# yas-sim/pyopenvino

Hardware: AMD Instinct MI355X
Metric: images/sec googlenet-v1 fp32 @batch256 (higher is better)
Workload: dtype f32

## Files before the change

include/pvhip.h:

```cpp
#ifndef PVHIP_H
#define PVHIP_H

#include <stddef.h>
#include <stdint.h>

#ifdef __cplusplus
extern "C" {
#endif

#define PVHIP_OK            0
#define PVHIP_EHIP         -1
#define PVHIP_EINVAL       -2
#define PVHIP_ENOTINIT     -3
#define PVHIP_ECOMM        -4
#define PVHIP_EUNSUPPORTED -5

#define PVHIP_ABI_VERSION   19

int         pvhip_abi_version(void);
const char* pvhip_last_error(void);
int         pvhip_device_count(int* count);
int         pvhip_init(int device);
int         pvhip_settings_reload(void);
int         pvhip_shutdown(void);
// ... 275 lines not shown
                                       int pad_top, int pad_left, int pad_bottom, int pad_right, int size, float alpha, float beta, float bias,
                                       int k_out, const float* conv_bias, int act);
int    pvhip_conv2d_f16_stem_supported(int c, int h, int w, int k_out, int kh, int kw, int sh, int sw, int pad_top, int pad_left, int oh, int ow);
size_t pvhip_conv2d_f16_stem_pack_elems(int k_out);
int    pvhip_conv2d_f16_stem_pack(const float* w_oihw, float* wf, int k_out);
int    pvhip_conv2d_f16_stem(const float* xp, const float* wf, void* yb, int n, int hp, int wp, int k_out, int oh, int ow,
                             const float* bias, int act);
int    pvhip_conv2d_f16_stem_direct_supported(int c, int h, int w, int k_out, int kh, int kw, int sh, int sw, int pad_top, int pad_left, int oh, int ow);
int    pvhip_conv2d_f16_stem_direct_pack(const float* w_oihw, float* wf, int k_out);
int    pvhip_conv2d_f16_stem_direct(const float* x, const float* wf, void* yb, int n, int h, int w, int k_out, int oh, int ow,
                                    const float* pre_add, const float* bias, int act);
int    pvhip_conv2d_stem_f32_supported(int c, int h, int w, int k_out, int kh, int kw, int sh, int sw, int pad_top, int pad_left, int oh, int ow);
size_t pvhip_conv2d_stem_f32_pack_elems(int k_out);
int    pvhip_conv2d_stem_f32_pack(const float* w_oihw, float* wf, int k_out);
int    pvhip_conv2d_stem_f32(const float* xp, const float* wf, float* y, int n, int hp, int wp, int k_out, int oh, int ow,
                             const float* bias, int act, float act_lo, float act_hi);
int    pvhip_conv2d_stem_direct_supported(int c, int h, int w, int k_out, int kh, int kw, int sh, int sw, int pad_top, int pad_left, int oh, int ow);
int    pvhip_conv2d_stem_direct_f32(const float* x, const float* wf, float* y, int n, int h, int w, int k_out, int oh, int ow,
                                    const float* pre_add, const float* bias, int act, float act_lo, float act_hi);
int    pvhip_conv2d_stem_direct_pool_supported(int n, int c, int h, int w, int k_out, int kh, int kw, int sh, int sw, int pad_top, int pad_left,
                                               int oh, int ow, int poh, int pow);
int    pvhip_conv2d_stem_direct_pool_f32(const float* x, const float* wf, float* y, float* yp, int n, int h, int w, int k_out, int oh, int ow,
                                         int poh, int pow, const float* pre_add, const float* bias, int act, float act_lo, float act_hi);
int    pvhip_conv2d_stem_wino_supported(int c, int h, int w, int k_out, int kh, int kw, int sh, int sw, int pad_top, int pad_left, int oh, int ow);
long   pvhip_conv2d_stem_wino_pack_elems(void);
int    pvhip_conv2d_stem_wino_pack(const float* w_oihw, float* u, int k_out);
int    pvhip_conv2d_stem_wino_f32(const float* x, const float* u, float* y, int n, int h, int w, int k_out, int oh, int ow,
                                  const float* pre_add, const float* bias, int act, float act_lo, float act_hi);
int    pvhip_avgpool_c8(const void* x, float* y, int n, int c, int h, int w, int oh, int ow, int kh, int kw, int sh, int sw);
int    pvhip_lrn_maxpool3x3_c8_supported(int h, int w, int oh, int ow, int sh, int sw, int pad_top, int pad_left, int size);
int    pvhip_lrn_maxpool3x3_c8(const void* x, void* y, int n, int c, int h, int w, int size, float alpha, float beta, float bias,
                               int oh, int ow, int sh, int sw, int pad_top, int pad_left, int pad_bottom, int pad_right);
int    pvhip_conv2d_f16_c8(const void* xb, const float* wf, float* y,
                           int n, int c, int h, int w, int k_out, int kh, int kw,
                           const float* bias, int act,
                           int out_channel_offset, int out_channels_total,
                           float act_lo, float act_hi);

int pvhip_dwconv2d_f32(const float* x, const float* w, float* y, int n, int g, int h, int wdt,
                       int kh, int kw, int oh, int ow, int sh, int sw, int pad_top, int pad_left,
                       const float* bias, int act, float act_lo, float act_hi);

int pvhip_detection_output_f32(const float* loc, const float* conf, const float* priors, float* out, int n,
                               int num_priors, int num_classes, int records_per_image, float confidence_threshold,
                               float nms_threshold, int code_type_center_size, int variance_encoded_in_target,
                               int clip_before_nms, int clip_after_nms);
// ... 144 lines not shown
```

pyopenvino_amd/csrc/pvhip_stem.hip:

```cpp
#include <type_traits>

#include "pvhip_common.h"

using namespace pvhip;

namespace {

typedef float    floatx4 __attribute__((ext_vector_type(4)));
typedef unsigned uintx4 __attribute__((ext_vector_type(4)));
typedef float    floatx2 __attribute__((ext_vector_type(2)));

constexpr int kC = 3, kKH = 7, kKW = 7, kST = 2, kPad = 3;
constexpr int kTR    = 4;
constexpr int kRows  = kST * (kTR - 1) + kKH;
constexpr int kLdsRow = 256;
constexpr int kCopies = kC * kRows;
constexpr int kBufBytes = kCopies * kLdsRow * 4;
constexpr int kTaps  = kC * kKH * kKW;
constexpr int kSteps = (kTaps + 3) / 4;
constexpr int kNG    = 7;
constexpr int kWaves = 2 * kTR;
constexpr int kThreads = kWaves * kWave;
constexpr bool kTransposeStores = true;
constexpr int kTsPitch = 116;
// ... 6 lines not shown
constexpr int kPoolLdsBytes = (kCarryBase + 64 * kHpCols) * 4;

struct StemArgs {
    const float* xp;
    const float* wf;
    float*       y;
    const float* bias;
    const float* pre_add;
    int N, HP, WP, OH, OW, K;
    int tiles_per_image, tiles;
    unsigned x_bytes, y_bytes;
    int act;
    float act_lo, act_hi;
    int tstores;
    float*   yp;
    int      POH, POW;
    unsigned yp_bytes;
};

__device__ __forceinline__ float lds_read_f32(unsigned addr) {
    return *reinterpret_cast<const __attribute__((address_space(3))) float*>(addr);
}

template <int ABL, bool DIRECT, bool POOL = false>
__global__ __launch_bounds__(kThreads, 1) void conv_stem_f32_kernel(StemArgs a) {
    static_assert(!POOL || (DIRECT && ABL == 0 && kTransposeStores), "the pooled output rides on the whole-row stores of the DIRECT form");
    extern __shared__ __attribute__((aligned(1024))) float stem_lds[];
    const int tid  = threadIdx.x;
    const int lane = tid & (kWave - 1);
    const int wid  = __builtin_amdgcn_readfirstlane(tid / kWave);
    const int hf = wid & 1, wr = wid >> 1;
    const int l15 = lane & 15, kq = lane >> 4;

    const int g_ = (int)gridDim.x, b_ = (int)blockIdx.x;
    const int per = a.tiles / g_, extra = a.tiles - per * g_;
    int       tile = b_ * per + min(b_, extra);
    const int tile_end = tile + per + (b_ < extra ? 1 : 0);
    if (tile >= tile_end) return;
    const int  tile_stop = tile_end + ((POOL && tile_end % a.tiles_per_image != 0) ? 1 : 0);
    bool       have_carry = false;

    const __amdgpu_buffer_rsrc_t xr = __builtin_amdgcn_make_buffer_rsrc(const_cast<float*>(a.xp), 0, a.x_bytes, 0x00020000);
    const __amdgpu_buffer_rsrc_t yr = __builtin_amdgcn_make_buffer_rsrc(a.y, 0, a.y_bytes, 0x00020000);

    float w[kSteps][2];
    {
        const float* const wp = a.wf + (size_t)hf * kSteps * 2 * kWave + lane;
#pragma unroll
        for (int m = 0; m < kSteps; ++m) {
// ... 111 lines not shown
        }
        lds_dma_wait_all();
        if (POOL) __syncthreads();
        if (ABL == 1) {
            floatx4 sum = acc[0][0];
#pragma unroll
            for (int g = 0; g < kNG; ++g) sum += acc[g][1] + (g ? acc[g][0] : acc[g][1]);
            if (sum[0] == 12345.678f) __builtin_amdgcn_raw_buffer_store_b128(__builtin_bit_cast(uintx4, sum), yr, (unsigned)(tid * 16), 0, 0);
        } else {
            const int img = tile / a.tiles_per_image;
            const int oy  = (tile - img * a.tiles_per_image) * kTR + wr;
            const unsigned plane = (unsigned)(a.OH * a.OW * 4);
            const unsigned rowb  = (unsigned)(((img * a.K + ch0) * a.OH + oy) * a.OW * 4 + 16 * kq);
            const bool rowok = oy < a.OH && !(POOL && tile >= tile_end);
            if (a.bias != nullptr) {
#pragma unroll
                for (int g = 0; g < kNG; ++g)
#pragma unroll
                    for (int t = 0; t < 2; ++t)
#pragma unroll
                        for (int r = 0; r < 4; ++r) acc[g][t][r] = acc[g][t][r] + bias_l[t];
            }
            auto store_all = [&]() {
                if (kTransposeStores && (POOL || a.tstores != 0)) {
                    float* const tl = stem_lds + kTsBase + wid * kTsWave;
                    const int c2 = lane / 28, q = lane - 28 * c2;
                    float* const hp0 = stem_lds + buf * (kCopies * kLdsRow) + 4 + wid * (16 * kHpCols);
                    int qe = q;
                    if (POOL) asm volatile("" : "+v"(qe));
                    qe = 4 * qe + 4 < a.OW ? 4 * qe + 4 : 4 * qe + 3;
#pragma unroll
                    for (int t = 0; t < 2; ++t) {
#pragma unroll
                        for (int g = 0; g < kNG; ++g) *reinterpret_cast<floatx4*>(tl + l15 * kTsPitch + 16 * g + 4 * kq) = acc[g][t];
                        floatx2 hp[8];
#pragma unroll
                        for (int p = 0; p < 8; ++p) {
                            const int ch = 32 * hf + 16 * t + 2 * p + c2;
                            const floatx4 v = *reinterpret_cast<const floatx4*>(tl + (2 * p + (c2 & 1)) * kTsPitch + 4 * q);
                            if (POOL) {
                                const float e = tl[(2 * p + (c2 & 1)) * kTsPitch + qe];
                                hp[p] = floatx2{max3_nan(v[0], v[1], v[2]), max3_nan(v[2], v[3], e)};
                            }
                            const bool ok = rowok && c2 < 2 && ch < a.K && 4 * q < a.OW;
                            const unsigned vo = ok ? (unsigned)(((img * a.K + ch) * a.OH + oy) * a.OW * 4 + 16 * q) : kOob;
                            __builtin_amdgcn_raw_buffer_store_b128(__builtin_bit_cast(uintx4, v), yr, vo, 0, 0);
// ... 403 lines not shown
                           {0.0f, 0.0f, 0.0f, 1.0f}};
    const int total = 4 * 3 * 36 * kWave;
    for (int e = blockIdx.x * blockDim.x + threadIdx.x; e < total; e += gridDim.x * blockDim.x) {
        const int lane = e & 63, p = (e >> 6) % 36, s = ((e >> 6) / 36) % 3, kg = (e >> 6) / 108;
        const int k = 16 * kg + (lane & 15), gq = lane >> 4, py = gq >> 1, px = gq & 1, pi = p / 6, pj = p - 6 * pi;
        float sum = 0.0f;
        if (k < K) {
            float row[4];
            for (int aa = 0; aa < 4; ++aa) {
                float r = 0.0f;
                for (int bb = 0; bb < 4; ++bb) {
                    const int ky = 2 * aa + py, kx = 2 * bb + px;
                    const float wv = (ky < kKH && kx < kKW) ? w[((size_t)(k * kC + s) * kKH + ky) * kKW + kx] : 0.0f;
                    r = __builtin_fmaf(wv, G[pj][bb], r);
                }
                row[aa] = r;
            }
            for (int aa = 0; aa < 4; ++aa) sum = __builtin_fmaf(G[pi][aa], row[aa], sum);
        }
        u[e] = sum;
    }
}

}

extern "C" {

int pvhip_conv2d_stem_f32_supported(int c, int h, int w, int k_out, int kh, int kw, int sh, int sw, int pad_top, int pad_left, int oh, int ow) {
    if (c != kC || kh != kKH || kw != kKW || sh != kST || sw != kST || pad_top != kPad || pad_left != kPad || k_out <= 0 || k_out > 64) return 0;
    if (h <= 0 || w <= 0 || oh <= 0 || ow <= 0 || ow > 16 * kNG || ow % 4 != 0) return 0;
    const int wp = (kST * (ow - 1) + kKW + 3) / 4 * 4;
    if (wp > kLdsRow || wp < w + kPad) return 0;
    return wp;
}

size_t pvhip_conv2d_stem_f32_pack_elems(int k_out) {
    if (k_out <= 0 || k_out > 64) return 0;
    return (size_t)2 * kSteps * 2 * kWave;
}

int pvhip_conv2d_stem_f32_pack(const float* w_oihw, float* wf, int k_out) {
    PVHIP_REQUIRE_INIT();
    PVHIP_CHECK_ARG(w_oihw != nullptr && wf != nullptr && k_out > 0 && k_out <= 64);
    hipLaunchKernelGGL(conv_stem_f32_pack_kernel, dim3(grid_for((size_t)2 * kSteps * 2 * kWave)), dim3(kBlock), 0, state().stream, w_oihw, wf, k_out);
    PVHIP_LAUNCH_CHECK();
    return PVHIP_OK;
// ... 43 lines not shown
    a.tiles_per_image = (oh + kTR - 1) / kTR;
    const long tiles = (long)n * a.tiles_per_image;
    if (tiles > 0x3fffffffL) return fail(PVHIP_EUNSUPPORTED, "pvhip_conv2d_stem_direct_f32: too many tiles");
    a.tiles = (int)tiles;
    a.x_bytes = (unsigned)in_b; a.y_bytes = (unsigned)out_b;
    a.act = act; a.act_lo = act_lo; a.act_hi = act_hi;
    return stem_launch<true>(a, tiles);
}

int pvhip_conv2d_stem_direct_pool_supported(int n, int c, int h, int w, int k_out, int kh, int kw, int sh, int sw, int pad_top, int pad_left, int oh, int ow,
                                            int poh, int pow) {
    if (!pvhip_conv2d_stem_direct_supported(c, h, w, k_out, kh, kw, sh, sw, pad_top, pad_left, oh, ow)) return 0;
    if (oh < 3 || ow < 4 || poh != (oh - 3 + 1) / 2 + 1 || pow != ow / 2) return 0;
    if (n < 0) return 0;
    if (n > 0) {
        const long tiles = (long)n * ((oh + kTR - 1) / kTR);
        if (tiles < (long)kPoolMinTiles * kNumCU) return 0;
    }
    return 1;
}

int pvhip_conv2d_stem_direct_pool_f32(const float* x, const float* wf, float* y, float* yp, int n, int h, int w, int k_out, int oh, int ow, int poh, int pow,
                                      const float* pre_add, const float* bias, int act, float act_lo, float act_hi) {
    PVHIP_REQUIRE_INIT();
    PVHIP_CHECK_ARG(n >= 0 && k_out > 0 && k_out <= 64 && h > 0 && w > 0 && oh > 0 && ow > 0 && act >= 0 && act <= 2);
    if (!pvhip_conv2d_stem_direct_pool_supported(0, kC, h, w, k_out, kKH, kKW, kST, kST, kPad, kPad, oh, ow, poh, pow))
        return fail(PVHIP_EUNSUPPORTED, "pvhip_conv2d_stem_direct_pool_f32: shape outside the kernel (ask pvhip_conv2d_stem_direct_pool_supported first)");
    const unsigned long long in_b = (unsigned long long)n * kC * h * w * 4ull, out_b = (unsigned long long)n * k_out * oh * ow * 4ull;
    if (in_b >= (1ull << 31) || out_b >= (1ull << 31)) return fail(PVHIP_EUNSUPPORTED, "pvhip_conv2d_stem_direct_pool_f32: tensor too large");
    if (n == 0) return PVHIP_OK;
    PVHIP_CHECK_ARG(x != nullptr && wf != nullptr && y != nullptr && yp != nullptr);
    StemArgs a;
    a.xp = x; a.wf = wf; a.y = y; a.bias = bias; a.pre_add = pre_add;
    a.N = n; a.HP = h; a.WP = w; a.OH = oh; a.OW = ow; a.K = k_out;
    a.tiles_per_image = (oh + kTR - 1) / kTR;
    const long tiles = (long)n * a.tiles_per_image;
    if (tiles > 0x3fffffffL) return fail(PVHIP_EUNSUPPORTED, "pvhip_conv2d_stem_direct_pool_f32: too many tiles");
    a.tiles = (int)tiles;
    a.x_bytes = (unsigned)in_b; a.y_bytes = (unsigned)out_b;
    a.act = act; a.act_lo = act_lo; a.act_hi = act_hi;
    a.tstores = 1;
    a.yp = yp; a.POH = poh; a.POW = pow; a.yp_bytes = (unsigned)((unsigned long long)n * k_out * poh * pow * 4ull);
    const int grid = (int)(tiles < kNumCU ? tiles : kNumCU);
    static bool attr_set = false;
    if (!attr_set) {
        PVHIP_HIP(hipFuncSetAttribute(reinterpret_cast<const void*>(conv_stem_f32_kernel<0, true, true>), hipFuncAttributeMaxDynamicSharedMemorySize, kPoolLdsBytes));
        attr_set = true;
    }
    hipLaunchKernelGGL((conv_stem_f32_kernel<0, true, true>), dim3((unsigned)grid), dim3(kThreads), (size_t)kPoolLdsBytes, state().stream, a);
    PVHIP_LAUNCH_CHECK();
    return PVHIP_OK;
}

int pvhip_conv2d_stem_wino_supported(int c, int h, int w, int k_out, int kh, int kw, int sh, int sw, int pad_top, int pad_left, int oh, int ow) {
    if (c != kC || kh != kKH || kw != kKW || sh != kST || sw != kST || pad_top != kPad || pad_left != kPad || k_out <= 0 || k_out > 64 || k_out % 16 != 0) return 0;
    if (h < 2 || w < 4 || h % 2 != 0 || w % 4 != 0 || w > 224 || oh != h / 2 || ow != w / 2) return 0;
    return 1;
}

long pvhip_conv2d_stem_wino_pack_elems(void) { return 4L * 3 * 36 * kWave; }

int pvhip_conv2d_stem_wino_pack(const float* w_oihw, float* u, int k_out) {
    PVHIP_REQUIRE_INIT();
    PVHIP_CHECK_ARG(w_oihw != nullptr && u != nullptr && k_out > 0 && k_out <= 64);
    hipLaunchKernelGGL(conv_stem_wino_pack_kernel, dim3(grid_for((size_t)4 * 3 * 36 * kWave)), dim3(kBlock), 0, state().stream, w_oihw, u, k_out);
    PVHIP_LAUNCH_CHECK();
    return PVHIP_OK;
}

int pvhip_conv2d_stem_wino_f32(const float* x, const float* u, float* y, int n, int h, int w, int k_out, int oh, int ow, const float* pre_add,
                               const float* bias, int act, float act_lo, float act_hi) {
    PVHIP_REQUIRE_INIT();
    PVHIP_CHECK_ARG(n >= 0 && act >= 0 && act <= 2);
    if (!pvhip_conv2d_stem_wino_supported(kC, h, w, k_out, kKH, kKW, kST, kST, kPad, kPad, oh, ow))
// ... 29 lines not shown
```

pyopenvino_amd/device.py:

```python
import ctypes
import os
import threading
import weakref

import numpy as np

_HERE = os.path.dirname(os.path.abspath(__file__))
LIB_PATH = os.path.join(_HERE, 'libpvhip.so')
DIAG_LIB_PATH = os.path.join(_HERE, 'libpvhip_diag.so')
if os.environ.get('PVHIP_LIBRARY'):
    LIB_PATH = os.path.abspath(os.environ['PVHIP_LIBRARY'])

MAX_RANK = 6
MAX_CONCAT = 16
UNIQUE_ID_BYTES = 128

_c = ctypes
_i64p = _c.POINTER(_c.c_int64)
_fp = _c.c_void_p

SIGNATURES = {
    'pvhip_abi_version': (_c.c_int, []),
    'pvhip_last_error': (_c.c_char_p, []),
    'pvhip_device_count': (_c.c_int, [_c.POINTER(_c.c_int)]),
# ... 90 lines not shown
    'pvhip_conv2d_f16_stem_supported': (_c.c_int, [_c.c_int] * 12),
    'pvhip_conv2d_f16_stem_pack_elems': (_c.c_size_t, [_c.c_int]),
    'pvhip_conv2d_f16_stem_pack': (_c.c_int, [_fp, _fp, _c.c_int]),
    'pvhip_conv2d_f16_stem': (_c.c_int, [_fp, _fp, _c.c_void_p] + [_c.c_int] * 6 + [_fp, _c.c_int]),
    'pvhip_conv2d_f16_stem_direct_supported': (_c.c_int, [_c.c_int] * 12),
    'pvhip_conv2d_f16_stem_direct_pack': (_c.c_int, [_fp, _fp, _c.c_int]),
    'pvhip_conv2d_f16_stem_direct': (_c.c_int, [_fp, _fp, _c.c_void_p] + [_c.c_int] * 6 + [_fp, _fp, _c.c_int]),
    'pvhip_conv2d_f16_dma_c8': (_c.c_int, [_fp, _fp, _c.c_void_p] + [_c.c_int] * 13 + [_fp, _c.c_int]),
    'pvhip_conv2d_f16_c8': (_c.c_int, [_c.c_void_p, _fp, _fp] + [_c.c_int] * 7 + [_fp, _c.c_int, _c.c_int, _c.c_int, _c.c_float, _c.c_float]),
    'pvhip_conv2d_kernel_kind': (_c.c_int, [_c.c_int] * 13),
    'pvhip_conv2d_form': (_c.c_int, [_c.c_int] * 14 + [_c.POINTER(_c.c_int)]),
    'pvhip_conv2d_stem_f32_supported': (_c.c_int, [_c.c_int] * 12),
    'pvhip_conv2d_stem_f32_pack_elems': (_c.c_size_t, [_c.c_int]),
    'pvhip_conv2d_stem_f32_pack': (_c.c_int, [_fp, _fp, _c.c_int]),
    'pvhip_conv2d_stem_f32': (_c.c_int, [_fp, _fp, _fp] + [_c.c_int] * 6 + [_fp, _c.c_int, _c.c_float, _c.c_float]),
    'pvhip_conv2d_stem_direct_supported': (_c.c_int, [_c.c_int] * 12),
    'pvhip_conv2d_stem_wino_supported': (_c.c_int, [_c.c_int] * 12),
    'pvhip_conv2d_stem_wino_pack_elems': (_c.c_long, []),
    'pvhip_conv2d_stem_wino_pack': (_c.c_int, [_fp, _fp, _c.c_int]),
    'pvhip_conv2d_stem_wino_f32': (_c.c_int, [_fp, _fp, _fp] + [_c.c_int] * 6 + [_fp, _fp, _c.c_int, _c.c_float, _c.c_float]),
    'pvhip_conv2d_stem_direct_f32': (_c.c_int, [_fp, _fp, _fp] + [_c.c_int] * 6 + [_fp, _fp, _c.c_int, _c.c_float, _c.c_float]),
    'pvhip_conv2d_stem_direct_pool_supported': (_c.c_int, [_c.c_int] * 15),
    'pvhip_conv2d_stem_direct_pool_f32': (_c.c_int, [_fp, _fp, _fp, _fp] + [_c.c_int] * 8 + [_fp, _fp, _c.c_int, _c.c_float, _c.c_float]),
    'pvhip_lrn_conv1x1_supported': (_c.c_int, [_c.c_int] * 4 + [_c.c_float] * 2 + [_c.c_int]),
    'pvhip_lrn_conv1x1_f32': (_c.c_int, [_fp, _fp, _fp] + [_c.c_int] * 4 + [_c.c_float] * 3 + [_c.c_int, _fp, _c.c_int, _c.c_float, _c.c_float]),
    'pvhip_conv2d_pooled_supported': (_c.c_int, [_c.c_int] * 5),
    'pvhip_conv2d_pooled_f32': (_c.c_int, [_fp, _fp, _fp] + [_c.c_int] * 5 + [_fp, _c.c_int, _c.c_int, _c.c_int, _c.c_float, _c.c_float]),
    'pvhip_conv2d_pooled_f16': (_c.c_int, [_fp, _fp, _fp] + [_c.c_int] * 5 + [_fp, _c.c_int, _c.c_int, _c.c_int, _c.c_float, _c.c_float]),
    'pvhip_conv2d_multi_supported': (_c.c_int, [_c.c_int] * 8),
    'pvhip_conv2d_multi_f32': (_c.c_int, [_fp, _fp] + [_c.c_int] * 12 + [_fp, _c.c_int, _c.c_float, _c.c_float, _c.c_int, _c.c_void_p]),
    'pvhip_conv2d_multi_f16_dma': (_c.c_int, [_fp, _fp] + [_c.c_int] * 12 + [_fp, _c.c_int, _c.c_float, _c.c_float, _c.c_int, _c.c_void_p]),
    'pvhip_dwconv2d_f32': (_c.c_int, [_fp, _fp, _fp] + [_c.c_int] * 12 + [_fp, _c.c_int, _c.c_float, _c.c_float]),
    'pvhip_detection_output_f32': (_c.c_int, [_c.c_void_p, _c.c_void_p, _c.c_void_p, _c.c_void_p, _c.c_int, _c.c_int, _c.c_int, _c.c_int,
                                              _c.c_float, _c.c_float, _c.c_int, _c.c_int, _c.c_int, _c.c_int]),
    'pvhip_detections_to_rois': (_c.c_int, [_c.c_void_p] * 4 + [_c.c_int] * 5 + [_c.c_float, _c.c_void_p, _c.c_int, _c.c_int, _c.c_int]),
    'pvhip_topk_rows_f32': (_c.c_int, [_c.c_void_p, _c.c_int, _c.c_int, _c.c_int, _c.c_void_p, _c.c_void_p]),
    'pvhip_detections_compact': (_c.c_int, [_c.c_void_p] + [_c.c_int] * 4 + [_c.c_float, _c.c_void_p] + [_c.c_int] * 4 + [_c.c_void_p] * 2),
    'pvhip_detections_compact_fit': (_c.c_int, [_c.c_void_p] + [_c.c_int] * 4 + [_c.c_float, _c.c_void_p] + [_c.c_int] * 4 + [_c.c_void_p] * 2 +
                                     [_c.c_int] * 6),
    'pvhip_detections_to_rois_fit': (_c.c_int, [_c.c_void_p] * 4 + [_c.c_int] * 5 + [_c.c_float, _c.c_void_p, _c.c_int, _c.c_int, _c.c_int] +
                                     [_c.c_int] * 6),
    'pvhip_detections_merge_tiles': (_c.c_int, [_c.c_void_p] * 2 + [_c.c_int] * 3 + [_c.c_float, _c.c_void_p] + [_c.c_int] * 5 + [_c.c_float] +
                                     [_c.c_int] * 2 + [_c.c_void_p] * 3),
    'pvhip_detections_merge_regions': (_c.c_int, [_c.c_void_p] * 2 + [_c.c_int] * 3 + [_c.c_float, _c.c_void_p] + [_c.c_int] * 5 + [_c.c_float] +
                                       [_c.c_int] * 5 + [_c.c_void_p] * 3),
    'pvhip_comm_unique_id': (_c.c_int, [_c.c_void_p]),
# ... 76 lines not shown
        fn = getattr(lib, name)
        fn.restype = restype
        fn.argtypes = argtypes
    _lib = lib
    return lib


def call(name, *args):
    lib = load_library()
    rc = getattr(lib, name)(*args)
    if name not in _NOT_STATUS and rc != 0:
        raise PvhipError('{} failed ({}): {}'.format(name, rc, lib.pvhip_last_error().decode(errors='replace')))
    return rc


def device_count() -> int:
    n = _c.c_int(0)
    lib = load_library()
    rc = lib.pvhip_device_count(_c.byref(n))
    return n.value if rc == 0 else 0


def init(device: int = None) -> int:
    global _initialised_device
    if device is None:
        device = int(os.environ.get('LOCAL_RANK', '0'))
        if device_count() == 1:
            device = 0
    if _initialised_device is not None:
        if _initialised_device != device:
            raise PvhipError('already bound to GPU {}'.format(_initialised_device))
        return device
    call('pvhip_init', int(device))
    _initialised_device = device
    return device


settings_serial = 0


def _env_level(name, default):
    try:
        return int(os.environ.get(name, default) or 0)
    except ValueError:
        return int(default)


def _plugin_settings():
    env = os.environ.get
    return {
        'conv_prepad': env('PVHIP_CONV_PREPAD', '1') != '0',
        'conv_f16_dma': env('PVHIP_CONV_F16_DMA', '1') != '0',
        'conv_f16_span': int(env('PVHIP_CONV_F16_SPAN', '1') or 0),
        'conv_stem_direct': env('PVHIP_CONV_STEM_DIRECT', '1') != '0',
        'conv_f16_stem': env('PVHIP_CONV_F16_STEM', '1') != '0',
        'conv_f16_c8': _env_level('PVHIP_CONV_F16_C8', '2'),
        'fuse_poolconv': _env_level('PVHIP_FUSE_POOLCONV', '2'),
        'fuse_stem_conv': _env_level('PVHIP_FUSE_STEM_CONV', '1'),
        'fuse_stem_pool': _env_level('PVHIP_FUSE_STEM_POOL', '1'),
    }


globals().update(_plugin_settings())


def reload_settings():
    global settings_serial
    call('pvhip_settings_reload')
    globals().update(_plugin_settings())
    settings_serial += 1


def ensure_init():
    if _initialised_device is None:
        init()


def is_initialised() -> bool:
    return _initialised_device is not None


def device_name() -> str:
    ensure_init()
    buf = ctypes.create_string_buffer(256)
    call('pvhip_device_name', buf, 256)
    return buf.value.decode()


def synchronize():
    ensure_init()
    call('pvhip_sync')


def shutdown():
    global _initialised_device, _pinned_total, _pinned_generation
    with _pinned_lock:
        _pinned_free.clear()
        _pinned_total = 0
        _pinned_generation += 1
    if _lib is not None and _initialised_device is not None:
        call('pvhip_shutdown')
    _initialised_device = None


def host_stats():
    a, b = _c.c_size_t(0), _c.c_size_t(0)
    call('pvhip_host_stats', _c.byref(a), _c.byref(b))
    return a.value, b.value


def current_device():
    return _initialised_device


def pool_stats():
    a, b = _c.c_size_t(0), _c.c_size_t(0)
    call('pvhip_pool_stats', _c.byref(a), _c.byref(b))
    return a.value, b.value


class _Block:
    __slots__ = ('ptr', 'nbytes')

    def __init__(self, nbytes: int):
        ensure_init()
# ... 140 lines not shown
                raise ValueError('cannot reshape tensor of size {} into shape {}'.format(self.size, tuple(shape)))
            shape[shape.index(-1)] = self.size // known
        n = 1
        for d in shape:
            n *= d
        if n != self.size:
            raise ValueError('cannot reshape tensor of size {} into shape {}'.format(self.size, tuple(shape)))
        return DeviceTensor(self._block, shape, self.dtype)

    def numpy(self) -> np.ndarray:
        out = _pinned_empty(self.shape, self.dtype)
        if out.nbytes:
            call('pvhip_memcpy_d2h', out.ctypes.data_as(_c.c_void_p), _c.c_void_p(self.ptr), out.nbytes)
        return out

    def __array__(self, dtype=None, copy=None):
        a = self.numpy()
        return a if dtype is None else a.astype(dtype, copy=False)

    def __repr__(self):
        return 'DeviceTensor(shape={}, dtype={}, ptr=0x{:x})'.format(self.shape, self.dtype.name, self.ptr)


class ChannelSlice:
    __slots__ = ('base', 'coff', 'shape', 'dtype')

    def __init__(self, base: DeviceTensor, coff: int, k: int):
        self.base, self.coff = base, int(coff)
        self.shape = (base.shape[0], int(k)) + tuple(base.shape[2:])
        self.dtype = base.dtype

    @property
    def ndim(self):
        return len(self.shape)

    @property
    def size(self):
        n = 1
        for d in self.shape:
            n *= d
        return n

    def numpy(self):
        return np.ascontiguousarray(self.base.numpy()[:, self.coff:self.coff + self.shape[1]])

    def __array__(self, dtype=None, copy=None):
# ... 83 lines not shown
    arr = (_c.c_int64 * max(1, len(values)))(*[int(v) for v in values])
    return arr


def pool_epoch_begin() -> int:
    ensure_init()
    e = _c.c_int(0)
    call('pvhip_pool_epoch_begin', _c.byref(e))
    return e.value


def pool_epoch_dispatched():
    call('pvhip_pool_epoch_dispatched')


def pool_epoch_end(epoch: int):
    call('pvhip_pool_epoch_end', int(epoch))


MAX_STREAMS = 9
COPY_STREAM = 8


def select_stream(index: int):
    ensure_init()
    call('pvhip_stream_select', int(index))


class Event:

    def __init__(self, timed: bool = True):
        ensure_init()
        h = _c.c_void_p(0)
        call('pvhip_event_create' if timed else 'pvhip_event_create_untimed', _c.byref(h))
        self.handle = h.value

    def wait(self):
        call('pvhip_stream_wait_event', _c.c_void_p(self.handle))
        return self

    def record(self):
        call('pvhip_event_record', _c.c_void_p(self.handle))
        return self

    def synchronize(self):
        call('pvhip_event_sync', _c.c_void_p(self.handle))

    def elapsed_ms(self, end: 'Event') -> float:
        ms = _c.c_float(0.0)
# ... 11 lines not shown
```

pyopenvino_amd/fusion_plan.py:

```python
import os

import numpy as np

from . import device

HINT_KEYS = ('_fuse_pool_in', '_pre_add', '_f16_mfma', '_fuse_bias', '_fuse_act', '_out_into', '_out_c8', '_siblings', '_fuse_pool',
             '_fuse_lrn', '_fuse_conv', '_fuse_pool_out', '_pooled_out', '_pooled_in')


def data_src(G, nid):
    return next((p_ for p_ in G.pred[nid] if G.edges[(p_, nid)]['connection'][3] == 0), None)


class FusionPlan:
    def __init__(self, G, order, f16=False):
        self.G = G
        self.order = list(order)
        self.f16 = f16
        self.fusion = {}
        self.fused_away = set()
        self.concat_direct = {}
        self.lrn_pool = {}
        self.siblings = {}
        self.pool_conv = {}
        self.pre_add = {}
        self.stem_conv = {}
        self.stem_pool = {}
        self.c8_out = set()
        self.c8_concat = set()
        self.c8_entry = set()
        self.receivers, self.owner, self.handed_on = {}, {}, {}

    def tail(self, cid):
        f = self.fusion[cid]
        return f['relu'] if f['relu'] is not None else f['add']

    def chain(self, cid):
        f = self.fusion[cid]
        return [n_ for n_ in (cid, f['add'], f['relu']) if n_ is not None]

    def _derive(self):
        self.receivers = {cid: [(0, n_) for n_ in self.chain(cid)[1:]] for cid in self.fusion if cid not in self.fused_away}
        for lead, sibs in self.siblings.items():
            self.receivers.setdefault(lead, []).extend((k, n_) for k, sid in enumerate(sibs, 1) for n_ in self.chain(sid))
        for lead, folded in self.lrn_pool.items():
            self.receivers.setdefault(lead, []).append((0, folded))
        for pid, cid in self.stem_conv.items():
            self.receivers.setdefault(pid, []).extend((0, n_) for n_ in self.chain(cid))
        self.owner = {n_: task for task, ports in self.receivers.items() for _, n_ in ports}
        self.handed_on = dict(list(self.pool_conv.values()) + [(add_id, src_id) for add_id, _, src_id in self.pre_add.values()])
# ... 194 lines not shown
        cid = readers[0]
        f = p.fusion.get(cid)
        if f is None or G.nodes[cid]['type'] != 'Convolution' or f['into'] is not None or any(cid in m for m in (p.siblings, p.fused_away, p.pool_conv, p.pre_add)):
            continue
        if pool.lrn_conv_fusable(G.nodes[pid], G.nodes[lid], G.nodes[cid]):
            p.stem_conv[pid] = cid
            p.fused_away.update(p.chain(cid))


def _stem_pool(p, plugins):
    G, conv, pool = p.G, plugins.get('Convolution'), plugins.get('MaxPool')
    if p.f16 or device.fuse_stem_pool == 0 or not getattr(conv, 'SUPPORTS_POOLED_OUTPUT', False) or not getattr(pool, 'SUPPORTS_POOLED_INPUT', False):
        return
    for cid, f in p.fusion.items():
        if G.nodes[cid]['type'] != 'Convolution' or f['into'] is not None or any(cid in m for m in (p.siblings, p.fused_away, p.pool_conv)):
            continue
        readers = list(G.successors(p.tail(cid)))
        if len(readers) != 1 or readers[0] not in p.stem_conv or G.edges[(p.tail(cid), readers[0])]['connection'][3] != 0:
            continue
        pid = readers[0]
        if conv.pooled_output_fusable(G.nodes[cid], G.nodes[pid], by_size=device.fuse_stem_pool != 2, pre_add=cid in p.pre_add) and \
                pool.pooled_input_ok(G.nodes[pid], G.nodes[p.lrn_pool[pid]], G.nodes[p.stem_conv[pid]]):
            p.stem_pool[cid] = pid


def _c8(conv, modules=False):
    on = device.conv_f16_c8 != 0 and device.conv_f16_dma and getattr(conv, 'SUPPORTS_C8', False)
    return bool(on) and (not modules or (device.conv_f16_c8 == 2 and getattr(conv, 'SUPPORTS_C8_MODULES', False)))


def _relu_or_none(f):
    return f['act'] is None or f['act'][0] == 'relu'


def _c8_writers(p, conv):
    G = p.G
    if not p.f16 or not _c8(conv):
        return
    for cid, f in p.fusion.items():
        if G.nodes[cid]['type'] != 'Convolution' or f['into'] is not None or cid in p.pool_conv or cid in p.pre_add or not _relu_or_none(f):
            continue
        tail = p.tail(cid)
        readers = list(G.successors(tail))
        if len(readers) != 1 or G.nodes[readers[0]]['type'] != 'Convolution' or G.edges[(tail, readers[0])]['connection'][3] != 0:
            continue
        rid = readers[0]
# ... 133 lines not shown
```

pyopenvino_amd/inference_engine.py:

```python
import contextlib
import copy
import ctypes
import importlib
import os
import pickle
import pkgutil
import sys
import time
import xml.etree.ElementTree as et

import networkx as nx
import numpy as np

from . import common_def, device, fusion_plan, stream_plan
from .answers import Answers
from .host_input import HostInputs
from .input_format import DetectedRois, InputInfo, PreProcessChannel, PreProcessInfo
from .stream_plan import CaptureStreamModel

DEFAULT_PLUGIN_PACKAGE = 'pyopenvino_amd.op_plugins'


class Plugins:

# ... 505 lines not shown

    def _order_event(self):
        event = self._order_events.pop() if self._order_events else device.Event(timed=False)
        self._events_in_flight.append(event)
        return event

    def run_tasks(self, verbose: bool = False):
        self._infer_serial += 1
        self._recycle_events()
        plan = self.plan_streams()
        epoch = None
        if plan is not None:
            self._order_events += self._events_in_flight
            self._events_in_flight = []
            epoch = device.pool_epoch_begin()
            device.select_stream(self.stream_base)
        try:
            self.last_node_times = self._dispatch_tasks(plan, epoch, verbose)
        except BaseException:
            if plan is not None:
                try:
                    device.select_stream(0)
                    device.synchronize()
                    device.pool_epoch_dispatched()
                    device.pool_epoch_end(epoch)
                except Exception:
                    pass
            raise

    def _dispatch_tasks(self, plan, epoch, verbose):
        G, registry, fp = self.ienet.G, self.ienet.ie.plugins.plugins, self.plan
        open_run, times = None, []
        if plan is not None:
            stream_of, waits, records = plan
            done_events, current, base = {}, 0, self.stream_base
            cap_model = CaptureStreamModel() if self._recording else None
            ops = self._stream_ops
        for task in fp.order:
            if task in fp.fused_away:
                continue
            node = G.nodes[task]
            node_type = node['type']
            if plan is not None and task in stream_of:
                if stream_of[task] != current:
                    current = stream_of[task]
                    device.select_stream(base + current)
# ... 91 lines not shown
            node['_fuse_bias'] = G.nodes[fusion['bias']]['output'][0]['data']
            node['_fuse_act'] = fusion['act']
            if fusion['into'] is not None:
                node['_out_into'] = (self._concat_buffer(fusion['into'][0]), fusion['into'][1])
        if task in fp.c8_out:
            node['_out_c8'] = True
        for sid in fp.siblings.get(task, ()):
            sf = fp.fusion[sid]
            node.setdefault('_siblings', []).append({'node': G.nodes[sid], 'inputs': self.prepare_inputs_for_task(sid),
                                                     'bias': G.nodes[sf['bias']]['output'][0]['data'], 'c8': sid in fp.c8_out,
                                                     'into': (self._concat_buffer(sf['into'][0]), sf['into'][1]) if sf['into'] is not None else None})
        folded = fp.lrn_pool.get(task)
        if folded is not None:
            node['_fuse_pool' if node['type'] == 'LRN' else '_fuse_lrn'] = G.nodes[folded]
        stem_conv = fp.stem_conv.get(task)
        if stem_conv is not None:
            sf = fp.fusion[stem_conv]
            wsrc = next(G.edges[(p_, stem_conv)]['connection'] for p_ in G.pred[stem_conv] if G.edges[(p_, stem_conv)]['connection'][3] == 1)
            node['_fuse_conv'] = {'node': G.nodes[stem_conv], 'w': G.nodes[wsrc[0]]['output'][wsrc[1]]['data'],
                                  'bias': G.nodes[sf['bias']]['output'][0]['data'], 'act': sf['act'], 'c8': fp.f16}
        pooled_by = fp.stem_pool.get(task)
        if pooled_by is not None:
            node['_fuse_pool_out'] = G.nodes[pooled_by]
        for cid, pid in fp.stem_pool.items():
            if pid == task:
                node['_pooled_in'] = G.nodes[cid].pop('_pooled_out', None)

    def capture_graph(self, inputs: dict, warm: int = 2, streams=1):
        if streams != 'plan':
            with _overridden(self, compute_streams=max(1, int(streams))):
                return self.capture_graph(inputs, warm=warm, streams='plan')
        G = self.ienet.G
        if not all(isinstance(v, device.DeviceTensor) for v in inputs.values()):
            raise ValueError('capture_graph needs device-resident inputs (DeviceTensor): their addresses go into the graph')
        self.release_graph()
        for _ in range(max(1, warm)):
            self._infer_eager(inputs)
        if self.recording_rings():
            raise device.PvhipError('capture_graph: this stream plan would close a ring in the runtime\'s parallel-stream lists '
                                    '(hipStreamEndCapture of ROCm 7.2 never returns from it); record on one stream')
        device.select_stream(self.stream_base)
        device.call('pvhip_graph_begin_capture')
        handle = ctypes.c_void_p()
        first_error = None
        try:
            with _overridden(self, device_timing=None, _recording=True), self._results_on_device():
                self.run_tasks(False)
        except BaseException as exc:
            first_error = exc
# ... 186 lines not shown
```

pyopenvino_amd/op_plugins/Convolution.py:

```python
import ctypes
from collections import namedtuple

import numpy as np

from .. import common_def
from .. import device as dev


SUPPORTS_FUSED_EPILOGUE = True
SUPPORTS_SIBLINGS = True
SUPPORTS_POOLED_INPUT = True
SUPPORTS_PRE_ADD = True
SUPPORTS_C8 = True
SUPPORTS_C8_MODULES = True


GRAPH_CAPTURE_SAFE = True

def name():
    print('Convolution')


def calc_output_shape(input_dim, kernel_dim, strides, pads_begin, pads_end, rounding_type, auto_pad):
    return tuple(common_def.pooled_extent(input_dim[i], kernel_dim[i], strides[i], pads_begin[i], pads_end[i],
# ... 352 lines not shown
    _check_channels(x, w)
    oh, ow = calc_output_shape((h, wd), (kh, kw), strides, pads_begin, pads_end, 'floor', auto_pad)
    hp, wp = h + pads_begin[0] + pads_end[0], wd + pads_begin[1] + pads_end[1]
    if oh > 0 and ow > 0 and ((oh - 1) * strides[0] + kh > hp or (ow - 1) * strides[1] + kw > wp):
        raise ValueError('could not broadcast input array: window exceeds the padded input '
                         '({}x{} padded, kernel {}x{}, stride {}, output {}x{})'.format(hp, wp, kh, kw, strides, oh, ow))
    pre_add = node.get('_pre_add')
    if pre_add is not None:
        pre_add = dev.as_device(pre_add)
        assert pre_add.size == c
    if r.label:
        node['_hip_f16'] = r.label
    act_code, act_lo, act_hi = dev.act_args(act)
    stem = _PACKERS[r.pack][2] == 1
    if stem:
        wpack = packed_weights(node, r.pack, w)
    if r.pad_row:
        xp = dev.DeviceTensor.empty((n, c, hp, r.pad_row))
        dev.call('pvhip_pad2d_f32', dev.ptr(x), dev.ptr(xp), n, c, h, wd, pads_begin[0], pads_begin[1], pads_end[0], r.pad_row - wd - pads_begin[1],
                 dev.ptr(pre_add))
        x, h, wd, pads_begin = xp, hp, r.pad_row, (0, 0)
    if not stem:
        wpack = packed_weights(node, r.pack, w, (h, wd) if r.pack in ('f32', 'f16') else ())
    target, coff, ctotal, y = _dest(into, n, kn, oh, ow, blocked=r.out == 'blocked')
    if stem:
        image = (dev.ptr(pre_add),) if r.entry in _IMAGE_READERS else ()
        epilogue = (act_code,) if r.out == 'blocked' else (act_code, act_lo, act_hi)
        pool_node = node.get('_fuse_pool_out')
        if pool_node is not None:
            node['_pooled_out'] = None
            pooled = _pooled_extent(pool_node, oh, ow) if r.entry == 'pvhip_conv2d_stem_direct_f32' and into is None else None
            if pooled is not None and dev.call('pvhip_conv2d_stem_direct_pool_supported', 0, c, h, wd, kn, kh, kw, *strides, *pads_begin, oh, ow, *pooled):
                yp = dev.DeviceTensor.empty((n, kn, pooled[0], pooled[1]))
                dev.call('pvhip_conv2d_stem_direct_pool_f32', dev.ptr(x), dev.ptr(wpack), dev.ptr(y), dev.ptr(yp), n, h, wd, kn, oh, ow, pooled[0], pooled[1],
                         dev.ptr(pre_add), dev.ptr(bias), act_code, act_lo, act_hi)
                node['_pooled_out'] = yp
                return y
        dev.call(r.entry, dev.ptr(x), dev.ptr(wpack), dev.ptr(y), n, h, wd, kn, oh, ow, *image, dev.ptr(bias), *epilogue)
    elif r.out == 'blocked':
        dev.call(r.entry, dev.ptr(x), dev.ptr(wpack), dev.ptr(y), n, c, h, wd, kn, kh, kw, oh, ow, strides[0], strides[1], pads_begin[0],
                 pads_begin[1], dev.ptr(bias), act_code)
    else:
        dev.call(r.entry, dev.ptr(x), dev.ptr(wpack), dev.ptr(target), n, c, h, wd, kn, kh, kw, oh, ow, strides[0], strides[1], pads_begin[0],
                 pads_begin[1], dev.ptr(bias), act_code, coff, ctotal, act_lo, act_hi)
    return y


def launch_c8(node, xb, w, bias=None, act=None, into=None):
    n, c, h, wd = xb.shape
    kn, _, kh, kw = w.shape
    _check_channels(xb, w)
    wpack = packed_weights(node, 'f16_c8', w)
    act_code, act_lo, act_hi = dev.act_args(act)
    target, coff, ctotal, y = _dest(into, n, kn, h, wd)
    node['_hip_f16'] = _label('pvhip_conv2d_f16_c8')
    dev.call('pvhip_conv2d_f16_c8', dev.ptr(xb), dev.ptr(wpack), dev.ptr(target), n, c, h, wd, kn, kh, kw, dev.ptr(bias), act_code, coff, ctotal,
             act_lo, act_hi)
    return y


# ... 110 lines not shown
```

Baseline: 56820.

## Skip writing full stem conv output when only the fused pool reads it

Adds a pool-only variant of the fused stem conv+maxpool kernel that writes just the pooled tensor and skips the full-resolution conv output. The full output is returned as a deferred tensor that recomputes the conv on demand if some consumer ever reads it. This removes a large global write (batch 256 x 64 x 112 x 112 fp32) from every pass. The cost is extra planner and runtime machinery, and a full recompute whenever the unpooled output is actually read, which is forbidden during graph capture.

```diff
diff --git a/include/pvhip.h b/include/pvhip.h
--- a/include/pvhip.h
+++ b/include/pvhip.h
@@ -321,6 +321,8 @@
                                                int oh, int ow, int poh, int pow);
 int    pvhip_conv2d_stem_direct_pool_f32(const float* x, const float* wf, float* y, float* yp, int n, int h, int w, int k_out, int oh, int ow,
                                          int poh, int pow, const float* pre_add, const float* bias, int act, float act_lo, float act_hi);
+int    pvhip_conv2d_stem_direct_poolonly_f32(const float* x, const float* wf, float* yp, int n, int h, int w, int k_out, int oh, int ow,
+                                             int poh, int pow, const float* pre_add, const float* bias, int act, float act_lo, float act_hi);
 int    pvhip_conv2d_stem_wino_supported(int c, int h, int w, int k_out, int kh, int kw, int sh, int sw, int pad_top, int pad_left, int oh, int ow);
 long   pvhip_conv2d_stem_wino_pack_elems(void);
 int    pvhip_conv2d_stem_wino_pack(const float* w_oihw, float* u, int k_out);
diff --git a/pyopenvino_amd/csrc/pvhip_stem.hip b/pyopenvino_amd/csrc/pvhip_stem.hip
--- a/pyopenvino_amd/csrc/pvhip_stem.hip
+++ b/pyopenvino_amd/csrc/pvhip_stem.hip
@@ -52,9 +52,10 @@
     return *reinterpret_cast<const __attribute__((address_space(3))) float*>(addr);
 }
 
-template <int ABL, bool DIRECT, bool POOL = false>
+template <int ABL, bool DIRECT, bool POOL = false, bool NOY = false>
 __global__ __launch_bounds__(kThreads, 1) void conv_stem_f32_kernel(StemArgs a) {
     static_assert(!POOL || (DIRECT && ABL == 0 && kTransposeStores), "the pooled output rides on the whole-row stores of the DIRECT form");
+    static_assert(!NOY || POOL, "without y the pooled tensor is the only output");
     extern __shared__ __attribute__((aligned(1024))) float stem_lds[];
     const int tid  = threadIdx.x;
     const int lane = tid & (kWave - 1);
@@ -212,6 +213,24 @@
                         for (int r = 0; r < 4; ++r) acc[g][t][r] = acc[g][t][r] + bias_l[t];
             }
             auto store_all = [&]() {
+                if constexpr (POOL && NOY) {
+                    float* const tl  = stem_lds + kTsBase + wid * kTsWave;
+                    float* const hp0 = stem_lds + buf * (kCopies * kLdsRow) + 4 + wid * (16 * kHpCols);
+                    const int from = ((lane + 16) & (kWave - 1)) * 4;
+#pragma unroll
+                    for (int t = 0; t < 2; ++t) {
+                        float* const row = (t == 0 ? hp0 + l15 * kHpCols : tl + l15 * kTsPitch) + 2 * kq;
+#pragma unroll
+                        for (int g = 0; g < kNG; ++g) {
+                            const floatx4 v = acc[g][t];
+                            const float pub = (g + 1 < kNG && kq == 0) ? acc[g + 1 < kNG ? g + 1 : g][t][0] : v[0];
+                            float e = __builtin_bit_cast(float, __builtin_amdgcn_ds_bpermute(from, __builtin_bit_cast(int, pub)));
+                            e = 16 * g + 4 * kq + 4 < a.OW ? e : v[3];
+                            *reinterpret_cast<floatx2*>(row + 8 * g) = floatx2{max3_nan(v[0], v[1], v[2]), max3_nan(v[2], v[3], e)};
+                        }
+                    }
+                    return;
+                }
                 if (kTransposeStores && (POOL || a.tstores != 0)) {
                     float* const tl = stem_lds + kTsBase + wid * kTsWave;
                     const int c2 = lane / 28, q = lane - 28 * c2;
@@ -661,6 +680,39 @@
     }
 }
 
+template <bool NOY>
+static int stem_pool_launch(const char* who, const float* x, const float* wf, float* y, float* yp, int n, int h, int w, int k_out, int oh, int ow, int poh,
+                            int pow, const float* pre_add, const float* bias, int act, float act_lo, float act_hi) {
+    PVHIP_REQUIRE_INIT();
+    PVHIP_CHECK_ARG(n >= 0 && k_out > 0 && k_out <= 64 && h > 0 && w > 0 && oh > 0 && ow > 0 && act >= 0 && act <= 2);
+    if (!pvhip_conv2d_stem_direct_pool_supported(0, kC, h, w, k_out, kKH, kKW, kST, kST, kPad, kPad, oh, ow, poh, pow))
+        return fail(PVHIP_EUNSUPPORTED, "%s: shape outside the kernel (ask pvhip_conv2d_stem_direct_pool_supported first)", who);
+    const unsigned long long in_b = (unsigned long long)n * kC * h * w * 4ull, out_b = (unsigned long long)n * k_out * oh * ow * 4ull;
+    if (in_b >= (1ull << 31) || out_b >= (1ull << 31)) return fail(PVHIP_EUNSUPPORTED, "%s: tensor too large", who);
+    if (n == 0) return PVHIP_OK;
+    PVHIP_CHECK_ARG(x != nullptr && wf != nullptr && (NOY || y != nullptr) && yp != nullptr);
+    StemArgs a;
+    a.xp = x; a.wf = wf; a.y = y; a.bias = bias; a.pre_add = pre_add;
+    a.N = n; a.HP = h; a.WP = w; a.OH = oh; a.OW = ow; a.K = k_out;
+    a.tiles_per_image = (oh + kTR - 1) / kTR;
+    const long tiles = (long)n * a.tiles_per_image;
+    if (tiles > 0x3fffffffL) return fail(PVHIP_EUNSUPPORTED, "%s: too many tiles", who);
+    a.tiles = (int)tiles;
+    a.x_bytes = (unsigned)in_b; a.y_bytes = NOY ? 0u : (unsigned)out_b;
+    a.act = act; a.act_lo = act_lo; a.act_hi = act_hi;
+    a.tstores = 1;
+    a.yp = yp; a.POH = poh; a.POW = pow; a.yp_bytes = (unsigned)((unsigned long long)n * k_out * poh * pow * 4ull);
+    const int grid = (int)(tiles < kNumCU ? tiles : kNumCU);
+    static bool attr_set = false;
+    if (!attr_set) {
+        PVHIP_HIP(hipFuncSetAttribute(reinterpret_cast<const void*>(conv_stem_f32_kernel<0, true, true, NOY>), hipFuncAttributeMaxDynamicSharedMemorySize, kPoolLdsBytes));
+        attr_set = true;
+    }
+    hipLaunchKernelGGL((conv_stem_f32_kernel<0, true, true, NOY>), dim3((unsigned)grid), dim3(kThreads), (size_t)kPoolLdsBytes, state().stream, a);
+    PVHIP_LAUNCH_CHECK();
+    return PVHIP_OK;
+}
+
 }
 
 extern "C" {
@@ -750,34 +802,13 @@
 
 int pvhip_conv2d_stem_direct_pool_f32(const float* x, const float* wf, float* y, float* yp, int n, int h, int w, int k_out, int oh, int ow, int poh, int pow,
                                       const float* pre_add, const float* bias, int act, float act_lo, float act_hi) {
-    PVHIP_REQUIRE_INIT();
-    PVHIP_CHECK_ARG(n >= 0 && k_out > 0 && k_out <= 64 && h > 0 && w > 0 && oh > 0 && ow > 0 && act >= 0 && act <= 2);
-    if (!pvhip_conv2d_stem_direct_pool_supported(0, kC, h, w, k_out, kKH, kKW, kST, kST, kPad, kPad, oh, ow, poh, pow))
-        return fail(PVHIP_EUNSUPPORTED, "pvhip_conv2d_stem_direct_pool_f32: shape outside the kernel (ask pvhip_conv2d_stem_direct_pool_supported first)");
-    const unsigned long long in_b = (unsigned long long)n * kC * h * w * 4ull, out_b = (unsigned long long)n * k_out * oh * ow * 4ull;
-    if (in_b >= (1ull << 31) || out_b >= (1ull << 31)) return fail(PVHIP_EUNSUPPORTED, "pvhip_conv2d_stem_direct_pool_f32: tensor too large");
-    if (n == 0) return PVHIP_OK;
-    PVHIP_CHECK_ARG(x != nullptr && wf != nullptr && y != nullptr && yp != nullptr);
-    StemArgs a;
-    a.xp = x; a.wf = wf; a.y = y; a.bias = bias; a.pre_add = pre_add;
-    a.N = n; a.HP = h; a.WP = w; a.OH = oh; a.OW = ow; a.K = k_out;
-    a.tiles_per_image = (oh + kTR - 1) / kTR;
-    const long tiles = (long)n * a.tiles_per_image;
-    if (tiles > 0x3fffffffL) return fail(PVHIP_EUNSUPPORTED, "pvhip_conv2d_stem_direct_pool_f32: too many tiles");
-    a.tiles = (int)tiles;
-    a.x_bytes = (unsigned)in_b; a.y_bytes = (unsigned)out_b;
-    a.act = act; a.act_lo = act_lo; a.act_hi = act_hi;
-    a.tstores = 1;
-    a.yp = yp; a.POH = poh; a.POW = pow; a.yp_bytes = (unsigned)((unsigned long long)n * k_out * poh * pow * 4ull);
-    const int grid = (int)(tiles < kNumCU ? tiles : kNumCU);
-    static bool attr_set = false;
-    if (!attr_set) {
-        PVHIP_HIP(hipFuncSetAttribute(reinterpret_cast<const void*>(conv_stem_f32_kernel<0, true, true>), hipFuncAttributeMaxDynamicSharedMemorySize, kPoolLdsBytes));
-        attr_set = true;
-    }
-    hipLaunchKernelGGL((conv_stem_f32_kernel<0, true, true>), dim3((unsigned)grid), dim3(kThreads), (size_t)kPoolLdsBytes, state().stream, a);
-    PVHIP_LAUNCH_CHECK();
-    return PVHIP_OK;
+    return stem_pool_launch<false>("pvhip_conv2d_stem_direct_pool_f32", x, wf, y, yp, n, h, w, k_out, oh, ow, poh, pow, pre_add, bias, act, act_lo, act_hi);
+}
+
+int pvhip_conv2d_stem_direct_poolonly_f32(const float* x, const float* wf, float* yp, int n, int h, int w, int k_out, int oh, int ow, int poh, int pow,
+                                          const float* pre_add, const float* bias, int act, float act_lo, float act_hi) {
+    return stem_pool_launch<true>("pvhip_conv2d_stem_direct_poolonly_f32", x, wf, nullptr, yp, n, h, w, k_out, oh, ow, poh, pow, pre_add, bias, act, act_lo,
+                                  act_hi);
 }
 
 int pvhip_conv2d_stem_wino_supported(int c, int h, int w, int k_out, int kh, int kw, int sh, int sw, int pad_top, int pad_left, int oh, int ow) {
diff --git a/pyopenvino_amd/device.py b/pyopenvino_amd/device.py
--- a/pyopenvino_amd/device.py
+++ b/pyopenvino_amd/device.py
@@ -136,6 +136,7 @@
     'pvhip_conv2d_stem_direct_f32': (_c.c_int, [_fp, _fp, _fp] + [_c.c_int] * 6 + [_fp, _fp, _c.c_int, _c.c_float, _c.c_float]),
     'pvhip_conv2d_stem_direct_pool_supported': (_c.c_int, [_c.c_int] * 15),
     'pvhip_conv2d_stem_direct_pool_f32': (_c.c_int, [_fp, _fp, _fp, _fp] + [_c.c_int] * 8 + [_fp, _fp, _c.c_int, _c.c_float, _c.c_float]),
+    'pvhip_conv2d_stem_direct_poolonly_f32': (_c.c_int, [_fp, _fp, _fp] + [_c.c_int] * 8 + [_fp, _fp, _c.c_int, _c.c_float, _c.c_float]),
     'pvhip_lrn_conv1x1_supported': (_c.c_int, [_c.c_int] * 4 + [_c.c_float] * 2 + [_c.c_int]),
     'pvhip_lrn_conv1x1_f32': (_c.c_int, [_fp, _fp, _fp] + [_c.c_int] * 4 + [_c.c_float] * 3 + [_c.c_int, _fp, _c.c_int, _c.c_float, _c.c_float]),
     'pvhip_conv2d_pooled_supported': (_c.c_int, [_c.c_int] * 5),
@@ -258,7 +259,7 @@
 
 
 def init(device: int = None) -> int:
-    global _initialised_device
+    global _initialised_device, _current_stream
     if device is None:
         device = int(os.environ.get('LOCAL_RANK', '0'))
         if device_count() == 1:
@@ -268,7 +269,7 @@
             raise PvhipError('already bound to GPU {}'.format(_initialised_device))
         return device
     call('pvhip_init', int(device))
-    _initialised_device = device
+    _initialised_device, _current_stream = device, 0
     return device
 
 
@@ -294,6 +295,7 @@
         'fuse_poolconv': _env_level('PVHIP_FUSE_POOLCONV', '2'),
         'fuse_stem_conv': _env_level('PVHIP_FUSE_STEM_CONV', '1'),
         'fuse_stem_pool': _env_level('PVHIP_FUSE_STEM_POOL', '1'),
+        'defer_stem_port': os.environ.get('PVHIP_DEFER_STEM_PORT', '1') != '0',
     }
 
 
@@ -329,14 +331,14 @@
 
 
 def shutdown():
-    global _initialised_device, _pinned_total, _pinned_generation
+    global _initialised_device, _pinned_total, _pinned_generation, _current_stream
     with _pinned_lock:
         _pinned_free.clear()
         _pinned_total = 0
         _pinned_generation += 1
     if _lib is not None and _initialised_device is not None:
         call('pvhip_shutdown')
-    _initialised_device = None
+    _initialised_device, _current_stream = None, 0
 
 
 def host_stats():
@@ -523,6 +525,32 @@
         return 'DeviceTensor(shape={}, dtype={}, ptr=0x{:x})'.format(self.shape, self.dtype.name, self.ptr)
 
 
+class DeferredTensor(DeviceTensor):
+    __slots__ = ('_make', '_real')
+
+    def __init__(self, shape, make, dtype=np.float32):
+        self.shape = tuple(int(d) for d in shape)
+        self.dtype = np.dtype(dtype)
+        self._make, self._real = make, None
+
+    @property
+    def materialised(self) -> bool:
+        return self._real is not None
+
+    @property
+    def _block(self):
+        if self._real is None:
+            real = self._make()
+            if not isinstance(real, DeviceTensor) or real.shape != self.shape or real.dtype != self.dtype:
+                raise PvhipError('a deferred tensor of {} {} was filled with {!r}'.format(self.shape, self.dtype.name, real))
+            self._real, self._make = real, None
+        return self._real._block
+
+    def __repr__(self):
+        return 'DeferredTensor(shape={}, dtype={}, {})'.format(self.shape, self.dtype.name,
+                                                               'ptr=0x{:x}'.format(self.ptr) if self.materialised else 'deferred')
+
+
 class ChannelSlice:
     __slots__ = ('base', 'coff', 'shape', 'dtype')
 
@@ -652,9 +680,18 @@
 COPY_STREAM = 8
 
 
+_current_stream = 0
+
+
 def select_stream(index: int):
+    global _current_stream
     ensure_init()
     call('pvhip_stream_select', int(index))
+    _current_stream = int(index)
+
+
+def current_stream() -> int:
+    return _current_stream
 
 
 class Event:
diff --git a/pyopenvino_amd/fusion_plan.py b/pyopenvino_amd/fusion_plan.py
--- a/pyopenvino_amd/fusion_plan.py
+++ b/pyopenvino_amd/fusion_plan.py
@@ -5,7 +5,7 @@
 from . import device
 
 HINT_KEYS = ('_fuse_pool_in', '_pre_add', '_f16_mfma', '_fuse_bias', '_fuse_act', '_out_into', '_out_c8', '_siblings', '_fuse_pool',
-             '_fuse_lrn', '_fuse_conv', '_fuse_pool_out', '_pooled_out', '_pooled_in')
+             '_fuse_lrn', '_fuse_conv', '_fuse_pool_out', '_pooled_out', '_pooled_in', '_defer_out')
 
 
 def data_src(G, nid):
@@ -26,6 +26,7 @@
         self.pre_add = {}
         self.stem_conv = {}
         self.stem_pool = {}
+        self.unread = set()
         self.c8_out = set()
         self.c8_concat = set()
         self.c8_entry = set()
@@ -266,6 +267,8 @@
         if conv.pooled_output_fusable(G.nodes[cid], G.nodes[pid], by_size=device.fuse_stem_pool != 2, pre_add=cid in p.pre_add) and \
                 pool.pooled_input_ok(G.nodes[pid], G.nodes[p.lrn_pool[pid]], G.nodes[p.stem_conv[pid]]):
             p.stem_pool[cid] = pid
+            if device.defer_stem_port and all(r_ == pid for n_ in p.chain(cid) for r_ in G.successors(n_) if r_ not in p.chain(cid)):
+                p.unread.add(cid)
 
 
 def _c8(conv, modules=False):
diff --git a/pyopenvino_amd/inference_engine.py b/pyopenvino_amd/inference_engine.py
--- a/pyopenvino_amd/inference_engine.py
+++ b/pyopenvino_amd/inference_engine.py
@@ -551,6 +551,9 @@
                 try:
                     device.select_stream(0)
                     device.synchronize()
+                except Exception:
+                    pass
+                try:
                     device.pool_epoch_dispatched()
                     device.pool_epoch_end(epoch)
                 except Exception:
@@ -688,9 +691,27 @@
         pooled_by = fp.stem_pool.get(task)
         if pooled_by is not None:
             node['_fuse_pool_out'] = G.nodes[pooled_by]
+            if task in fp.unread:
+                node['_defer_out'] = self._late_launch
         for cid, pid in fp.stem_pool.items():
             if pid == task:
                 node['_pooled_in'] = G.nodes[cid].pop('_pooled_out', None)
+
+    def _late_launch(self, run):
+        if self._recording:
+            raise device.PvhipError('a deferred port cannot be read while a pass is being recorded (capture_graph): read it after the capture')
+        before = device.current_stream()
+        device.select_stream(self.stream_base)
+        done = None
+        try:
+            out = run()
+            if before != self.stream_base:
+                done = device.Event(timed=False).record()
+            return out
+        finally:
+            device.select_stream(before)
+            if done is not None:
+                done.wait()
 
     def capture_graph(self, inputs: dict, warm: int = 2, streams=1):
         if streams != 'plan':
diff --git a/pyopenvino_amd/op_plugins/Convolution.py b/pyopenvino_amd/op_plugins/Convolution.py
--- a/pyopenvino_amd/op_plugins/Convolution.py
+++ b/pyopenvino_amd/op_plugins/Convolution.py
@@ -398,20 +398,29 @@
         x, h, wd, pads_begin = xp, hp, r.pad_row, (0, 0)
     if not stem:
         wpack = packed_weights(node, r.pack, w, (h, wd) if r.pack in ('f32', 'f16') else ())
+    pool_node = node.get('_fuse_pool_out') if stem else None
+    if pool_node is not None:
+        node['_pooled_out'] = None
+        pooled = _pooled_extent(pool_node, oh, ow) if r.entry == 'pvhip_conv2d_stem_direct_f32' and into is None else None
+        if pooled is not None and dev.call('pvhip_conv2d_stem_direct_pool_supported', 0, c, h, wd, kn, kh, kw, *strides, *pads_begin, oh, ow, *pooled):
+            yp = node['_pooled_out'] = dev.DeviceTensor.empty((n, kn, pooled[0], pooled[1]))
+            operands = (n, h, wd, kn, oh, ow), (dev.ptr(pre_add), dev.ptr(bias), act_code, act_lo, act_hi)
+            late = node.get('_defer_out')
+            if late is None:
+                y = dev.DeviceTensor.empty((n, kn, oh, ow))
+                dev.call('pvhip_conv2d_stem_direct_pool_f32', dev.ptr(x), dev.ptr(wpack), dev.ptr(y), dev.ptr(yp), *operands[0], *pooled, *operands[1])
+                return y
+            dev.call('pvhip_conv2d_stem_direct_poolonly_f32', dev.ptr(x), dev.ptr(wpack), dev.ptr(yp), *operands[0], *pooled, *operands[1])
+
+            def fill(held=(x, wpack, pre_add, bias)):
+                y = dev.DeviceTensor.empty((n, kn, oh, ow))
+                dev.call('pvhip_conv2d_stem_direct_f32', dev.ptr(held[0]), dev.ptr(held[1]), dev.ptr(y), *operands[0], *operands[1])
+                return y
+            return dev.DeferredTensor((n, kn, oh, ow), lambda: late(fill))
     target, coff, ctotal, y = _dest(into, n, kn, oh, ow, blocked=r.out == 'blocked')
     if stem:
         image = (dev.ptr(pre_add),) if r.entry in _IMAGE_READERS else ()
         epilogue = (act_code,) if r.out == 'blocked' else (act_code, act_lo, act_hi)
-        pool_node = node.get('_fuse_pool_out')
-        if pool_node is not None:
-            node['_pooled_out'] = None
-            pooled = _pooled_extent(pool_node, oh, ow) if r.entry == 'pvhip_conv2d_stem_direct_f32' and into is None else None
-            if pooled is not None and dev.call('pvhip_conv2d_stem_direct_pool_supported', 0, c, h, wd, kn, kh, kw, *strides, *pads_begin, oh, ow, *pooled):
-                yp = dev.DeviceTensor.empty((n, kn, pooled[0], pooled[1]))
-                dev.call('pvhip_conv2d_stem_direct_pool_f32', dev.ptr(x), dev.ptr(wpack), dev.ptr(y), dev.ptr(yp), n, h, wd, kn, oh, ow, pooled[0], pooled[1],
-                         dev.ptr(pre_add), dev.ptr(bias), act_code, act_lo, act_hi)
-                node['_pooled_out'] = yp
-                return y
         dev.call(r.entry, dev.ptr(x), dev.ptr(wpack), dev.ptr(y), n, h, wd, kn, oh, ow, *image, dev.ptr(bias), *epilogue)
     elif r.out == 'blocked':
         dev.call(r.entry, dev.ptr(x), dev.ptr(wpack), dev.ptr(y), n, c, h, wd, kn, kh, kw, oh, ow, strides[0], strides[1], pads_begin[0],
```

After: 56980, median of 2. Within noise of the previous version (+0.3%).
